# pucedoteth/dora

Measured on AMD Instinct MI355X. Metric: node->node GB/s (40,960,000 B UInt8 samples) + p50/p99 latency per msg size, higher is better.
Workload: dtype u8; 1 GPU; C2: examples/benchmark node->sink edge, device-resident UInt8 samples, 1 node + 1 sink per GPU; msg_bytes=40960000, parallelism=dp1 (one dataflow per GPU)

## Files before the change

### dora_amd/_lib.py

```python
from __future__ import annotations

import ctypes
import os
from ctypes import (POINTER, c_char_p, c_double, c_float, c_int, c_int32, c_int64, c_size_t,
                    c_uint8, c_uint32, c_uint64, c_void_p)

from .arrow_c import ArrowArray, ArrowSchema

LIB_DIR = os.path.join(os.path.dirname(os.path.abspath(__file__)), "lib")
LIB_PATH = os.path.join(LIB_DIR, "libdora_gpu.so")
TESTING_PATH = os.path.join(LIB_DIR, "libdora_gpu_testing.so")

ARROW_DEVICE_CPU = 1
ARROW_DEVICE_ROCM = 10
ARROW_DEVICE_ROCM_HOST = 11

DORA_OK = 0
ERRORS = {-1: "invalid", -2: "hip", -3: "too_small", -4: "unsupported", -5: "closed",
          -6: "timeout", -7: "not_found"}


class DoraGpuError(RuntimeError):
    def __init__(self, code, msg):
        super().__init__(f"[{ERRORS.get(code, code)}] {msg}")
# ... 254 lines not shown
                                        POINTER(c_int), POINTER(c_int), POINTER(c_float),
                                        POINTER(c_uint64), POINTER(c_uint64), POINTER(c_uint64)]),
    "dora_gpu_test_plan_quant": (c_int, [c_void_p, c_size_t, POINTER(c_int), POINTER(c_int),
                                         POINTER(c_int), POINTER(c_int)]),
    "dora_gpu_test_plan_take": (c_int, [c_void_p, POINTER(c_int), POINTER(c_void_p),
                                        POINTER(c_uint64), POINTER(c_uint64), POINTER(c_int),
                                        POINTER(ctypes.c_int64), POINTER(ctypes.c_int64),
                                        POINTER(ctypes.c_int64)]),
    "dora_gpu_test_plan_mask": (c_int, [c_void_p, POINTER(c_int), POINTER(c_void_p),
                                        POINTER(c_uint64), POINTER(ctypes.c_int64),
                                        POINTER(ctypes.c_int64), POINTER(c_uint64),
                                        POINTER(c_uint64), POINTER(ctypes.c_int64)]),
    "dora_gpu_test_plan_launch": (c_int, [c_void_p, POINTER(c_int), POINTER(c_int),
                                          POINTER(c_int)]),
    "dora_gpu_test_aql_hold": (c_int, [c_int, c_int]),
    "dora_gpu_test_reduce_timeout": (c_int, [c_uint64]),
    "dora_gpu_test_d2h_copy_probe": (c_int, [c_int, c_int, c_uint64, c_uint32, c_uint64, c_void_p]),
    "dora_gpu_test_stream_order_probe": (c_int, [c_int, c_int, c_uint64, c_uint32, c_void_p]),
    "dora_gpu_test_abandoned_slots": (c_int, [c_int, POINTER(c_uint32)]),
    "dora_gpu_test_publish_kernel": (c_int, [c_void_p, c_size_t, c_uint64, POINTER(FillTicket),
                                             c_uint32, c_uint32, c_void_p]),
    "dora_gpu_test_keep_awake_stats": (c_int, [c_int, POINTER(c_uint64), POINTER(c_int)]),
    "dora_gpu_test_aql_ring_wc": (c_int, [c_int, ctypes.POINTER(c_int), ctypes.POINTER(c_int)]),
    "dora_gpu_test_bcast_group": (c_int, [c_int, c_void_p, c_uint64, POINTER(c_int),
                                          POINTER(c_int)]),
    "dora_gpu_test_l1_stale": (c_int, [c_int, c_int, POINTER(c_uint32), POINTER(c_uint32),
                                       POINTER(c_uint32)]),
    "dora_gpu_test_ide_output": (c_int, [c_char_p, c_char_p, c_char_p, c_void_p, c_size_t,
                                         c_void_p, c_size_t, c_uint64, c_uint64, c_void_p,
                                         c_void_p, c_size_t, c_int, c_void_p, c_size_t,
# ... 69 lines not shown
```

### dora_amd/csrc/aql.cpp

```cpp
#include "aql.h"

#include <hip/hip_runtime_api.h>
#include <hsa/hsa.h>
#include <hsa/amd_hsa_signal.h>
#include <hsa/hsa_ext_amd.h>
#include <immintrin.h>
#include <pthread.h>
#include <sys/prctl.h>

#include <algorithm>
#include <chrono>
#include <condition_variable>
#include <cstdio>
#include <cstdlib>
#include <cstring>
#include <deque>
#include <mutex>
#include <string>
#include <thread>
#include <vector>

#include "common.h"
#include "shm.h"

// ... 214 lines not shown
}

void on_queue_error(hsa_status_t st, hsa_queue_t*, void* data) {
  const char* m = nullptr;
  hsa_status_string(st, &m);
  std::fprintf(stderr, "dora-gpu: AQL pack queue error: %s\n", m ? m : "?");
  static_cast<AqlQueue*>(data)->failed.store(true);
}

AqlQueue* create(int device) {
  auto note = [&](const char* what) {
    if (std::getenv("DORA_GPU_TRACE"))
      std::fprintf(stderr, "dora-gpu: AQL dispatch off on device %d: %s\n", device, what);
    return nullptr;
  };
  int bus = 0, dev = 0, dom = 0;
  if (hipDeviceGetAttribute(&bus, hipDeviceAttributePciBusId, device) != hipSuccess ||
      hipDeviceGetAttribute(&dev, hipDeviceAttributePciDeviceId, device) != hipSuccess ||
      hipDeviceGetAttribute(&dom, hipDeviceAttributePciDomainID, device) != hipSuccess)
    return note("PCI location");
  if (hsa_init() != HSA_STATUS_SUCCESS) return note("hsa_init");
  Agents f;
  f.bdf = (uint32_t(bus) << 8) | (uint32_t(dev) << 3);
  f.domain = uint32_t(dom);
  hsa_iterate_agents(on_agent, &f);
  if (!f.gpu_ok || !f.cpu_ok) return note("agent");
  if (f.matches != 1) return note("several GPU agents at the device's PCI location");
  hsa_amd_agent_iterate_memory_pools(f.gpu, on_pool, &f);
  if (!f.pool_ok) return note("device memory pool");
  auto* a = new AqlQueue();
  a->gpu = f.gpu;
  a->device = device;
  hsa_amd_hdp_flush_t hdp{};
  if (hsa_agent_get_info(f.gpu, static_cast<hsa_agent_info_t>(HSA_AMD_AGENT_INFO_HDP_FLUSH),
                         &hdp) != HSA_STATUS_SUCCESS ||
      !hdp.HDP_MEM_FLUSH_CNTL) {
    delete a;
    return note("HDP flush register");
  }
  a->hdp = hdp.HDP_MEM_FLUSH_CNTL;
  hsa_code_object_reader_t reader;
  hsa_executable_t exe;
  const size_t co_size = size_t(dora_aql_code_object_end - dora_aql_code_object);
  if (hsa_code_object_reader_create_from_memory(dora_aql_code_object, co_size, &reader) !=
          HSA_STATUS_SUCCESS ||
      hsa_executable_create_alt(HSA_PROFILE_FULL, HSA_DEFAULT_FLOAT_ROUNDING_MODE_DEFAULT,
                                nullptr, &exe) != HSA_STATUS_SUCCESS ||
      hsa_executable_load_agent_code_object(exe, f.gpu, reader, nullptr, nullptr) !=
          HSA_STATUS_SUCCESS ||
      hsa_executable_freeze(exe, nullptr) != HSA_STATUS_SUCCESS) {
    delete a;
    return note("code object");
  }
  for (int k = 0; k < kKernels; ++k) {
    hsa_executable_symbol_t sym;
    uint32_t ka = 0;
    const std::string sym_name = std::string(kKernelNames[k]) + ".kd";
    if (hsa_executable_get_symbol_by_name(exe, sym_name.c_str(), &f.gpu, &sym) != HSA_STATUS_SUCCESS ||
        hsa_executable_symbol_get_info(sym, HSA_EXECUTABLE_SYMBOL_INFO_KERNEL_OBJECT,
                                       &a->kobj[k]) != HSA_STATUS_SUCCESS ||
        hsa_executable_symbol_get_info(sym, HSA_EXECUTABLE_SYMBOL_INFO_KERNEL_KERNARG_SEGMENT_SIZE,
                                       &ka) != HSA_STATUS_SUCCESS ||
        hsa_executable_symbol_get_info(sym, HSA_EXECUTABLE_SYMBOL_INFO_KERNEL_GROUP_SEGMENT_SIZE,
                                       &a->group[k]) != HSA_STATUS_SUCCESS ||
        hsa_executable_symbol_get_info(
            sym, HSA_EXECUTABLE_SYMBOL_INFO_KERNEL_PRIVATE_SEGMENT_SIZE, &a->priv[k]) !=
            HSA_STATUS_SUCCESS ||
        ka != (k == kMultiKernel    ? aql_args_size()
               : k == kBatchKernel  ? aql_batch_args_size()
               : k == kReduceKernel ? size_t(kReduceArgsBytes)
               : k == kReadKernel   ? size_t(kReadArgsBytes)
                                    : size_t(kArgs1Bytes)) ||
        ka > kSlotBytes) {
      delete a;
      return note("kernel symbol / argument size");
    }
  }
  void* ring = nullptr;
  if (hsa_amd_memory_pool_allocate(f.pool, size_t(kRingSlots) * kSlotBytes, 0, &ring) !=
          HSA_STATUS_SUCCESS ||
      hsa_amd_agents_allow_access(1, &f.cpu, nullptr, ring) != HSA_STATUS_SUCCESS) {
    delete a;
    return note("argument ring");
  }
  a->ring = static_cast<uint8_t*>(ring);
  std::vector<uint8_t> zero(kSlotBytes, 0);
  for (uint32_t r = 0; r < kRingSlots; ++r)
    std::memcpy(a->ring + size_t(r) * kSlotBytes, zero.data(), kSlotBytes);
  __builtin_ia32_sfence();
  (void)*reinterpret_cast<volatile uint32_t*>(a->ring + size_t(kRingSlots - 1) * kSlotBytes);
  const int create_queues = std::min(kMaxQueues, kQueues);
  for (int i = 0; i < create_queues; ++i) {
    if (hsa_queue_create(f.gpu, kQueuePackets, HSA_QUEUE_TYPE_SINGLE, on_queue_error, a,
                         UINT32_MAX, UINT32_MAX, &a->qs[i]) != HSA_STATUS_SUCCESS)
      break;
    a->nq = i + 1;
  }
  if (a->nq > 0) {
    hsa_amd_pointer_info_t pi{};
    pi.size = sizeof(pi);
    if (hsa_amd_pointer_info(a->qs[0]->base_address, &pi, nullptr, nullptr, nullptr) ==
        HSA_STATUS_SUCCESS) {
      const int owner = pi.agentOwner.handle == f.cpu.handle   ? 1
                        : pi.agentOwner.handle == f.gpu.handle ? 2
                        : pi.agentOwner.handle                  ? 3
                                                                : 0;
      a->ring_where = int(pi.type) * 4 + owner;
      a->wc_ring = owner == 2;
    }
  }
  if (a->nq == 0) {
    hsa_amd_memory_pool_free(ring);
    delete a;
    return note("queue");
  }
  hsa_amd_agent_iterate_memory_pools(f.cpu, on_cpu_pool, &f);
  void* hr = nullptr;
  if (f.kernarg_ok &&
      hsa_amd_memory_pool_allocate(f.kernarg, size_t(kRingSlots) * kHostSlotBytes, 0, &hr) ==
          HSA_STATUS_SUCCESS) {
    if (hsa_amd_agents_allow_access(1, &f.gpu, nullptr, hr) == HSA_STATUS_SUCCESS) {
      std::memset(hr, 0, size_t(kRingSlots) * kHostSlotBytes);
      a->hring = static_cast<uint8_t*>(hr);
    } else {
      hsa_amd_memory_pool_free(hr);
    }
  }
  hsa_system_get_info(HSA_SYSTEM_INFO_TIMESTAMP_FREQUENCY, &a->ts_freq);
  a->cpu = f.cpu;
  std::pair<hsa_amd_memory_pool_t, bool> coarse{{}, false};
  hsa_amd_agent_iterate_memory_pools(f.gpu, on_coarse_pool, &coarse);
  a->coarse = coarse.first;
  a->coarse_ok = coarse.second;
  return a;
}

}

namespace {
void warm_main(AqlQueue* a);
void stop_warm_threads();
std::mutex g_queues_mu;
AqlQueue* g_queues[64] = {};
}

AqlQueue* aql_queue(int device) {
  static std::mutex& mu = g_queues_mu;
  static AqlQueue** queues = g_queues;
  static bool tried[64] = {};
  if (device < 0 || device >= 64) return nullptr;
  std::lock_guard<std::mutex> g(mu);
  if (!tried[device]) {
    tried[device] = true;
    queues[device] = create(device);
    if (queues[device]) {
      queues[device]->warm_thread = std::thread(warm_main, queues[device]);
      static std::once_flag once;
      std::call_once(once, [] {
        std::atexit(stop_warm_threads);
        pthread_atfork(nullptr, nullptr, [] {
          for (AqlQueue* q : g_queues)
            if (q && q->warm_thread.joinable()) {
              new (&q->warm_thread) std::thread();
              q->warm_stop.store(true);
            }
        });
      });
    }
  }
  AqlQueue* q = queues[device];
  return (q && !q->failed.load()) ? q : nullptr;
}

bool aql_usable(const AqlQueue* q) { return q && !q->failed.load(std::memory_order_relaxed); }

size_t aql_max_segments() { return 8; }

namespace {
void drain_backlog(AqlQueue* a, std::chrono::steady_clock::time_point t0,
                   std::chrono::steady_clock::duration limit) {
  for (;;) {
    {
      std::lock_guard<std::mutex> g(a->mu);
      if (a->backlog.empty() || a->failed.load()) return;
    }
    if (std::chrono::steady_clock::now() - t0 > limit) return;
    std::this_thread::yield();
  }
// ... 8 lines not shown
  }
  const auto t0 = std::chrono::steady_clock::now();
  for (AqlQueue* a : qs) {
    if (!a) continue;
    drain_backlog(a, t0, std::chrono::seconds(5));
    std::lock_guard<std::mutex> g(a->mu);
    if (a->fallback) (void)hipStreamSynchronize(a->fallback);
    for (Use& u : a->uses)
      while (u.flag && !fill_reached(u.flag, u.epoch) &&
             std::chrono::steady_clock::now() - t0 < std::chrono::seconds(5))
        __builtin_ia32_pause();
  }
}

void aql_forget_flags(int device, const void* base, size_t size) {
  AqlQueue* a = aql_queue(device);
  if (!a) return;
  const auto t0 = std::chrono::steady_clock::now();
  drain_backlog(a, t0, std::chrono::seconds(2));
  std::lock_guard<std::mutex> g(a->mu);
  if (a->fallback) (void)hipStreamSynchronize(a->fallback);
  const auto* lo = static_cast<const uint8_t*>(base);
  std::deque<Pending> keep_backlog;
  for (const Pending& p : a->backlog) {
    const auto* f = reinterpret_cast<const uint8_t*>(p.flag_host);
    if (f < lo || f >= lo + size) keep_backlog.push_back(p);
  }
  a->backlog.swap(keep_backlog);
  for (auto& o : a->outq) {
    std::deque<Use> keep;
    for (const Use& u : o) {
      const auto* f = reinterpret_cast<const uint8_t*>(u.flag);
// ... 823 lines not shown
```

### dora_amd/csrc/aql.h

```cpp
#pragma once

#include <atomic>
#include <cstddef>
#include <cstdint>

#include "plan.h"

namespace dora {

struct AqlQueue;

AqlQueue* aql_queue(int device);
bool aql_usable(const AqlQueue* q);

int aql_pack(AqlQueue* q, const Segment* segs, size_t n, uint8_t* dst, const FillSignal& sig,
             const std::atomic<uint64_t>* flag_host, bool profile, uint64_t dst_cap = 0,
             uint64_t* cp_stamps = nullptr, bool sync = false, bool* read_signalled = nullptr);
bool aql_cp_candidate(const Segment* segs, size_t n, bool lone = false);

void aql_forget_flags(int device, const void* base, size_t size);

void aql_fence_all();

size_t aql_kernel_count();
const char* aql_kernel_name(size_t k);
uint64_t aql_dispatched(int device, size_t k);
int aql_hold(int device, bool hold);
// ... 29 lines not shown
```

### dora_amd/csrc/node.cpp

```cpp
#include "node_internal.h"

namespace dora {
namespace {

constexpr uint64_t kDropWaitNs = 10000000000;

bool numa_pinning() {
  static const bool v = [] {
    const char* e = std::getenv("DORA_GPU_PIN");
    return !(e && *e == '0');
  }();
  return v;
}

int gpu_numa_node(int device) {
  char bus[64] = {0};
  if (hipDeviceGetPCIBusId(bus, sizeof(bus), device) != hipSuccess) return -1;
  for (char* p = bus; *p; ++p) *p = char(std::tolower(*p));
  const std::string path = std::string("/sys/bus/pci/devices/") + bus + "/numa_node";
  FILE* f = std::fopen(path.c_str(), "r");
  if (!f) return -1;
  int numa = -1;
  if (std::fscanf(f, "%d", &numa) != 1) numa = -1;
  std::fclose(f);
// ... 68 lines not shown
    hipStream_t st = nullptr;
    if (hipStreamCreateWithFlags(&st, hipStreamNonBlocking) != hipSuccess) {
      (void)hipGetLastError();
      c->bcast_error = "broadcast stream of output `" + o + "`";
      continue;
    }
    if (bcast_join(uid, static_cast<int>(nranks), 0, 30000, &comm) == DORA_OK) {
      n->bcast_out[o] = {comm, st};
    } else {
      c->bcast_error = dora_gpu_last_error();
      (void)hipStreamDestroy(st);
    }
  }
}

}
}

extern "C" {

int dora_node_init(const char* shm_name, const char* node_id, int device, dora_node** out) {
  if (!shm_name || !node_id || !out) return dora::fail(DORA_ERR_INVALID, "NULL argument");
  *out = nullptr;
  DORA_GUARD_BEGIN
  auto core = std::make_shared<dora::NodeCore>();
  try {
    core->region.reset(dora::Region::attach(shm_name));
  } catch (const std::exception& e) {
    return dora::fail(DORA_ERR_INVALID, "attach dataflow: %s", e.what());
  }
  core->idx = core->region->node_index(node_id);
// ... 43 lines not shown
    }
  }

  auto* n = new dora_node();
  n->pin_pending = device < 0 && dora::numa_pinning();
  if (const char* e = std::getenv("DORA_GPU_SEND_ASYNC")) n->async_default = *e == '1';
  n->core = core;
  n->id = node_id;
  for (auto& o : dora::split(e.outputs, ',')) n->outputs.insert(o);
  for (auto& kv : dora::split(e.inputs, ',')) {
    auto eq = kv.find('=');
    n->queue_size[kv.substr(0, eq)] = static_cast<uint32_t>(std::stoul(kv.substr(eq + 1)));
  }
  n->min_queue_size = SIZE_MAX;
  for (auto& kv : n->queue_size) n->min_queue_size = std::min<size_t>(n->min_queue_size, kv.second);
  int rc = core->request(dora::REQ_SUBSCRIBE, {});
  if (rc != DORA_OK) {
    delete n;
    return rc;
  }
  const uint64_t t0 = dora::mono_ns();
  for (;;) {
    uint32_t kind;
    std::vector<uint8_t> p;
    if (core->ev.try_pop(&kind, &p)) {
      if (kind == dora::EV_READY) {
        if (p.size() >= 4) {
          dora::RBuf r(p);
          for (uint32_t k = r.u32(); k > 0; --k) n->host_bound.insert(r.str());
        }
// ... 32 lines not shown
  const char* shm = std::getenv("DORA_GPU_DATAFLOW");
  const char* id = std::getenv("DORA_NODE_ID");
  const char* dev = std::getenv("DORA_GPU_DEVICE");
  if (!shm || !id)
    return dora::fail(DORA_ERR_INVALID,
                      "env variables DORA_GPU_DATAFLOW and DORA_NODE_ID must be set. Are you sure "
                      "the node was started by the dataflow launcher?");
  return dora_node_init(shm, id, dev ? std::atoi(dev) : 0, out);
}

void dora_node_free(dora_node* n) {
  if (!n) return;
  struct Flush {
    ~Flush() { dora::trace_flush(); }
  } flush_trace_at_end;
  dora::stdout_capture_stop(n->stdout_capture);
  n->stdout_capture = nullptr;
  dora::stop_pump(n);
  std::vector<std::string> outs(n->outputs.begin(), n->outputs.end());
  dora::WBuf w;
  w.u32(static_cast<uint32_t>(outs.size()));
  for (auto& o : outs) w.str(o);
  (void)n->core->request(dora::REQ_CLOSE_OUTPUTS, w.data(), w.size());
  n->queue.clear();
  uint64_t t0 = dora::mono_ns();
  while (!n->sent_out.empty() || !n->forwarded.empty()) {
    dora::handle_finished_drop_tokens(n);
    if (n->sent_out.empty() && n->forwarded.empty()) break;
    if (dora::mono_ns() - t0 > dora::kDropWaitNs) break;
    n->core->drops.wait(10000);
// ... 153 lines not shown
```

### dora_amd/csrc/node_internal.h

```cpp

#pragma once
#include <hip/hip_runtime_api.h>
#include <pthread.h>
#include <unistd.h>
#include <x86intrin.h>

#include <algorithm>
#include <chrono>
#include <atomic>
#include <condition_variable>
#include <cstdio>
#include <cstdlib>
#include <cstring>
#include <deque>
#include <map>
#include <memory>
#include <memory_resource>
#include <mutex>
#include <new>
#include <thread>
#include <set>
#include <sstream>
#include <random>
#include <string>
// ... 80 lines not shown
  uint64_t cap = 0;
  uint64_t id = 0;
  hipIpcMemHandle_t handle;
  int flag = -1;
  uint64_t fill_epoch = 0;
  uint64_t region_epoch = 0;
  int region_cp_area = -1;
  hipEvent_t done = nullptr;
  hipIpcEventHandle_t done_handle;
  hipEvent_t use_ev = nullptr;
  bool use_pending = false;
  bool host = false;
  std::string shm_name;
  bool registered = false;
  bool bar = false, bar_tried = false;
};

inline uint64_t slot_bytes(uint64_t len) {
  constexpr uint64_t kSlotGrain = 2ull << 20;
  return (std::max<uint64_t>(len, 1) + kSlotGrain - 1) / kSlotGrain * kSlotGrain;
}

constexpr size_t kFillStreams = 1;

constexpr uint64_t kTimingPeriod = 8;

enum PeerCopyMode { PEER_KERNEL, PEER_SDMA };

struct OwnSlots {
  std::mutex mu;
// ... 422 lines not shown
  std::vector<uint32_t> cp_used;
  hipEvent_t start = nullptr;
  std::vector<hipEvent_t> stop;
  uint64_t packs = 0, bytes = 0;
  void fold(uint64_t a, uint64_t b) {
    if (!a || b < a) return;
    if (!stamped || a < tmin) tmin = a;
    if (!stamped || b > tmax) tmax = b;
    ++stamped;
    if (ticks.size() < 2 * (1u << 16)) {
      ticks.push_back(a);
      ticks.push_back(b);
    }
  }
  ~TimedRegion();
};

struct PlanCache {
  struct Entry {
    std::vector<uint64_t> key;
    dora_plan* plan = nullptr;
    std::vector<uint8_t> ti;
    uint64_t last_use = 0;
  };
  std::vector<Entry> entries;
  std::unordered_map<uint64_t, size_t> index;
  std::vector<uint64_t> key_buf;
  uint64_t clock = 0, hits = 0;
  static uint64_t hash(const std::vector<uint64_t>& key) {
    return fnv1a_words(key.data(), key.size());
// ... 38 lines not shown
  std::unordered_set<dora_sample*> samples_live;
  std::thread pump;
  std::mutex qmu;
  std::condition_variable qcv;
  std::atomic<bool> pump_on{false}, pump_stop{false};
  bool want_pump = false;
  bool pin_pending = false;
  dora::TimedRegion timed;
  dora::PackTiming prof;
  dora::PlanCache plans;
  uint64_t aql_packs = 0, hip_packs = 0;
  uint64_t bar_fills = 0;
  std::set<std::string, std::less<>> host_bound;
  uint64_t host_packs = 0, host_copies = 0;
  bool aql_ready = false;
  uint64_t slots_created = 0, cache_hits = 0, dropped_inputs = 0;
  std::vector<uint8_t> drop_buf;
  std::vector<uint8_t> ev_buf;
  bool compact = false;
  bool async_default = false;
  struct BcastOut {
    dora::BcastComm* comm = nullptr;
    hipStream_t stream = nullptr;
  };
  std::map<std::string, BcastOut> bcast_out;
  uint64_t bcast_seq = 0;
  dora::StdoutCapture* stdout_capture = nullptr;
  std::unordered_map<dora::DropToken, std::shared_ptr<dora::InputData>, dora::DropTokenHash>
      forwarded;
  uint64_t zero_copy_forwards = 0;
// ... 11 lines not shown
  if (note == NOTE_NONE) return;
  const std::atomic<uint64_t>* f = c->flag_host(s->slot->flag);
  if (note == NOTE_SYNC_AND_FENCE) NodeCore::note(c->aql_pending, f, epoch);
  NodeCore::note(c->flag_pending, f, epoch);
}

void release_slot_memory(Slot* s);
int self_pid();
bool wait_slot_idle(dora_node* n, Slot* s, uint64_t timeout_ns = kFillWaitNs);
void free_slot(dora_node* n, Slot* s);
void drain_slot_reaper();
void add_to_cache(dora_node* n, Slot* s);
void on_token(dora_node* n, const DropToken& t);
int handle_finished_drop_tokens(dora_node* n);
int allocate_slot(dora_node* n, uint64_t len, Slot** out);
int allocate_host_slot(dora_node* n, uint64_t len, Slot** out);
void discard_sample(dora_node* n, dora_sample* s);
dora_sample* vec_sample(const uint8_t* p, size_t len);
int proxy_send(dora_node* n, const char* output_id, const uint8_t* ti, size_t ti_len,
               const uint8_t* params, size_t params_len, dora_sample* sample, uint64_t ts);
PeerCopyMode peer_copy_mode();
bool edge_copy_forced();
int ensure_peer_access(NodeCore* c, int src_device);
int enqueue_peer_copy(NodeCore* c, void* dst, const void* src, int src_device, uint64_t len);
int ensure_local(InputData* in);
void encode_event(dora_node* n, uint32_t kind, const std::vector<uint8_t>& p);
void start_pump(dora_node* n);
void stop_pump(dora_node* n);
void harvest_region_stamp(dora_node* n, Slot* s);
void ensure_cp_stamps(dora_node* n);

}
```

### dora_amd/csrc/node_measure.cpp

```cpp

#include "node_internal.h"

namespace dora {

void harvest_region_stamp(dora_node* n, Slot* s) {
  const FillFlag& ff = n->core->region->hdr()->nodes[n->core->idx].fill[s->flag];
  if (s->region_cp_area >= 0 && ff.epoch.load(std::memory_order_acquire) != s->region_epoch &&
      ff.cp_epoch.load(std::memory_order_acquire) == s->region_epoch) {
    n->timed.cp_used.push_back(uint32_t(s->region_cp_area));
  } else if (ff.epoch.load(std::memory_order_acquire) == s->region_epoch) {
    n->timed.fold(ff.t_start, ff.t_end);
  }
  s->region_epoch = 0;
  s->region_cp_area = -1;
}

void ensure_cp_stamps(dora_node* n) {
  if (n->timed.cp_stamps || n->core->device < 0) return;
  const size_t bytes = size_t(kRegionCpAreas) * kCpAreaWords * 8;
  void* d = nullptr;
  if (bar_alloc(n->core->device, bytes, &d) != DORA_OK) {
    clear_error();
    return;
  }
  const std::vector<uint8_t> zero(bytes, 0);
  if (bar_write(n->core->device, d, zero.data(), bytes) != DORA_OK) {
    bar_free(d);
    clear_error();
    return;
  }
  n->timed.cp_stamps = static_cast<uint64_t*>(d);
  void* idx = nullptr;
  void* out = nullptr;
  if (hipHostMalloc(&idx, kRegionCpAreas * 4, hipHostMallocCoherent) == hipSuccess &&
      hipHostMalloc(&out, kRegionCpAreas * 16, hipHostMallocCoherent) == hipSuccess) {
    n->timed.reduce_idx = static_cast<uint32_t*>(idx);
    n->timed.reduce_out = static_cast<uint64_t*>(out);
  } else {
    (void)hipGetLastError();
    if (idx) (void)hipHostFree(idx);
  }
}

constexpr size_t kTimingPairs = 64;
constexpr size_t kMaxIntervals = 1 << 16;

void PackTiming::harvest(TimingPair& p) {
  if (!p.pending) return;
  float ms = 0;
  if (hipEventSynchronize(p.stop) == hipSuccess &&
      hipEventElapsedTime(&ms, p.start, p.stop) == hipSuccess) {
    pack_ms += ms;
    ++pack_count;
    pack_bytes += p.bytes;
    float a = 0, b = 0;
    if (timing_ref && intervals.size() < 2 * kMaxIntervals &&
// ... 237 lines not shown
```

### dora_amd/csrc/node_recv.cpp

```cpp

#include "node_internal.h"

namespace dora {

PeerCopyMode peer_copy_mode() {
  static const PeerCopyMode v = [] {
    const char* e = std::getenv("DORA_GPU_PEER_COPY");
    return (e && std::string(e) == "sdma") ? PEER_SDMA : PEER_KERNEL;
  }();
  return v;
}

bool edge_copy_forced() {
  static const bool v = [] {
    const char* e = std::getenv("DORA_GPU_EDGE_COPY");
    return e && *e && *e != '0';
  }();
  return v;
}

namespace {

void join_bcast_group(dora_node* n, const std::string& input, const uint8_t* uid, uint32_t nranks,
                      uint32_t rank) {
// ... 112 lines not shown
          auto it = own_slots().ptrs.find(d.ipc.slot_id);
          if (it != own_slots().ptrs.end()) base = it->second;
        } else {
          IpcKey key;
          std::memcpy(key.b, d.ipc.handle, 64);
          key.pid = d.ipc.owner_pid;
          key.slot = d.ipc.slot_id;
          NodeCore* c = n->core.get();
          std::lock_guard<std::mutex> g(c->ipc_mu);
          auto it = c->ipc_cache.find(key);
          if (it != c->ipc_cache.end()) {
            in->mapping = it->second;
          } else {
            hipIpcMemHandle_t h;
            std::memcpy(&h, d.ipc.handle, sizeof(h));
            DeviceScope ds(c->device >= 0 ? c->device : int(d.ipc.device));
            hipError_t e = hipIpcOpenMemHandle(&base, h, hipIpcMemLazyEnablePeerAccess);
            if (e != hipSuccess) {
              ev->type = DORA_EVENT_ERROR;
              ev->error = std::string("hipIpcOpenMemHandle: ") + hipGetErrorString(e) +
                          " (slot " + std::to_string(d.ipc.slot_id) + " of pid " +
                          std::to_string(d.ipc.owner_pid) + " on GPU " +
                          std::to_string(d.ipc.device) + ", " + std::to_string(d.ipc.len) + " B)";
              base = nullptr;
            } else {
              in->mapping = std::make_shared<IpcMapping>();
              in->mapping->base = base;
              c->ipc_cache.emplace(key, in->mapping);
              c->ipc_opens.fetch_add(1, std::memory_order_relaxed);
              n->core->region->hdr()->nodes[c->idx].ipc_opens.fetch_add(1, std::memory_order_relaxed);
              c->trim_ipc_cache();
// ... 29 lines not shown
      const uint32_t rank = r.u32();
      join_bcast_group(n, input, uid, nranks, rank);
      return;
    }
    default:
      return;
  }
  n->queue.push_back(std::move(ev));
}

namespace {

int stage_to_host(InputData* in, int src_device) {
  NodeCore* c = in->core.get();
  if (in->ext_len) {
    DeviceScope ds(src_device);
    uint64_t cap = 0;
    void* h = c->host_pool.get(in->ext_len, &cap);
    if (!h)
      return fail(DORA_ERR_HIP, "pinned staging buffer of %llu bytes",
                  (unsigned long long)in->ext_len);
    hipError_t e = hipSuccess;
    const int hrc = hsa_copy_host(h, in->ptr, in->ext_len, true);
    if (hrc == DORA_ERR_TIMEOUT) return hrc;
    if (hrc != DORA_OK) {
      static std::atomic<bool> noted{false};
      if (std::getenv("DORA_GPU_TRACE") && !noted.exchange(true))
        std::fprintf(stderr, "dora-gpu: staging through HIP's copy: %s\n", dora_gpu_last_error());
      clear_error();
      hipStream_t st = c->stage_stream(src_device);
      e = st ? hipMemcpyAsync(h, in->ptr, in->ext_len, hipMemcpyDeviceToHost, st)
             : hipErrorInvalidResourceHandle;
      if (e == hipSuccess) e = hipStreamSynchronize(st);
    }
    if (e != hipSuccess) {
      (void)hipGetLastError();
      c->host_pool.put(h, cap);
// ... 450 lines not shown
```

### dora_amd/csrc/node_send.cpp

```cpp

#include "node_internal.h"

namespace dora {
namespace {

constexpr uint64_t kSmallInFlightBytes = 8ull << 20;

size_t max_in_flight(uint64_t len) {
  static const std::pair<long, long> env = [] {
    const char* e = std::getenv("DORA_GPU_MAX_IN_FLIGHT");
    if (!e) return std::make_pair(0L, 0L);
    char* end = nullptr;
    const long a = std::strtol(e, &end, 10);
    const long b = (end && *end == ':') ? std::atol(end + 1) : a;
    return std::make_pair(a, b);
  }();
  const long v = len < kSmallInFlightBytes ? env.first : env.second;
  if (v > 0) return static_cast<size_t>(v);
  return len < kSmallInFlightBytes ? 11 : 8;
}

constexpr uint64_t kSlotWaitNs = 5000000;

void put_metadata(WBuf& w, const std::vector<uint8_t>& ti, const uint8_t* params,
// ... 129 lines not shown
    return DORA_OK;
  }
  if (n->core->device < 0 || (host_inline && std::max(len, ext_len) < kZeroCopyThreshold)) {
    auto* s = new dora_sample();
    s->len = len;
    s->vec.assign(len, 0);
    *out = s;
    return DORA_OK;
  }
  SubSpan sp_new(SP_SAMPLE_NEW);
  auto* s = new dora_sample();
  s->len = len;
  sp_new.stop();
  if (len > 0) {
    if (!n->aql_ready) {
      n->aql_ready = true;
      if (aql_queue(n->core->device)) ensure_cp_stamps(n);
    }
    SubSpan sp_tok(SP_ALLOC_TOKENS);
    handle_finished_drop_tokens(n);
    sp_tok.stop();
    SubSpan sp_wait(SP_ALLOC_WAIT);
    wait_for_send_credit(n, len);
    sp_wait.stop();
    s->ext_len = std::max(len, ext_len);
    SubSpan sp_slot(SP_ALLOC_SLOT);
    int rc = allocate_slot(n, s->ext_len + workspace, &s->slot);
    if (rc != DORA_OK) {
      delete s;
      return rc;
    }
  }
// ... 801 lines not shown
```

### dora_amd/csrc/node_slots.cpp

```cpp

#include "node_internal.h"

namespace dora {
namespace {

constexpr size_t kMaxCacheSize = 20;
constexpr size_t kMaxCacheSlots = 64;
uint64_t slot_cache_bytes() {
  static const uint64_t v = [] {
    const char* e = std::getenv("DORA_GPU_SLOT_CACHE_BYTES");
    return e ? std::strtoull(e, nullptr, 10) : uint64_t(4) << 30;
  }();
  return v;
}

}

void release_slot_memory(Slot* s) {
  if (s->host) {
    if (s->registered) (void)hipHostUnregister(s->ptr);
    shmem_unmap(s->ptr, s->cap);
    shmem_unlink(s->shm_name);
  } else {
    if (s->done) (void)hipEventDestroy(s->done);
// ... 178 lines not shown
    }
  }
  return best;
}

int allocate_slot(dora_node* n, uint64_t len, Slot** out) {
  const int best = best_fit(n, len, slot_bytes(len), false);
  if (best >= 0) {
    Slot* s = n->cache[static_cast<size_t>(best)];
    n->cache.erase(n->cache.begin() + best);
    SubSpan sp_flag(SP_SLOT_FLAG);
    const bool idle = wait_slot_idle(n, s);
    sp_flag.stop();
    if (idle) {
      *out = s;
      ++n->cache_hits;
      return DORA_OK;
    }
    std::fprintf(stderr, "dora-gpu: slot %llu: last fill did not complete; not reused\n",
                 (unsigned long long)s->id);
    std::lock_guard<std::mutex> g(own_slots().mu);
    own_slots().ptrs.erase(s->id);
  }
  auto* s = new Slot();
  s->cap = slot_bytes(len);
  s->id = own_slots().next_id.fetch_add(1);
  DeviceScope ds(n->core->device);
  hipError_t e = hipMalloc(&s->ptr, slot_bytes(len));
  if (e == hipSuccess) e = hipIpcGetMemHandle(&s->handle, s->ptr);
  if (e == hipSuccess) {
    if (n->core->region_dev && !n->core->free_flags.empty()) {
      s->flag = static_cast<int>(n->core->free_flags.back());
      n->core->free_flags.pop_back();
    } else {
      e = hipEventCreateWithFlags(&s->done, hipEventInterprocess | hipEventDisableTiming);
      if (e == hipSuccess) e = hipIpcGetEventHandle(&s->done_handle, s->done);
    }
  }
  if (e != hipSuccess) {
    if (s->flag >= 0) n->core->free_flags.push_back(static_cast<uint32_t>(s->flag));
    if (s->done) (void)hipEventDestroy(s->done);
    if (s->ptr) (void)hipFree(s->ptr);
    delete s;
    return fail(DORA_ERR_HIP, "device slot of %llu bytes: %s", (unsigned long long)len,
                hipGetErrorString(e));
  }
  {
    std::lock_guard<std::mutex> g(own_slots().mu);
    own_slots().ptrs[s->id] = s->ptr;
  }
  ++n->slots_created;
  n->core->region->hdr()->nodes[n->core->idx].slots_created.fetch_add(1, std::memory_order_relaxed);
  *out = s;
  return DORA_OK;
}

int allocate_host_slot(dora_node* n, uint64_t len, Slot** out) {
  constexpr uint64_t kPage = 4096;
  const uint64_t need = (std::max<uint64_t>(len, 1) + kPage - 1) / kPage * kPage;
  const int best = best_fit(n, len, need, true);
  if (best >= 0) {
    *out = n->cache[static_cast<size_t>(best)];
    n->cache.erase(n->cache.begin() + best);
    ++n->cache_hits;
    return DORA_OK;
  }
  auto* s = new Slot();
  s->host = true;
  s->cap = need;
// ... 23 lines not shown
```

### dora_amd/csrc/subprof.h

```cpp
#pragma once

#include <x86intrin.h>

#include <cstdint>

namespace dora {

enum SubPhase : int {
  SP_SEND_PLAN = 0,
  SP_ALLOC_TOKENS,
  SP_ALLOC_WAIT,
  SP_ALLOC_SLOT,
  SP_STREAM_QUERY,
  SP_AQL_PACK,
  SP_AQL_ARGS,
  SP_AQL_DISPATCH,
  SP_SEND_TI,
  SP_SEND_TOKENS,
  SP_SEND_LOOKUP,
  SP_SEND_REQUEST,
  SP_SEND_TRACK,
  SP_RECV_DRAIN,
  SP_RECV_ENCODE,
  SP_RECV_DROPOLD,
// ... 9 lines not shown
extern const bool g_subprof_on;
inline bool subprof_enabled() { return g_subprof_on; }
void subprof_add(int phase, uint64_t ticks);

struct SubSpan {
  int phase;
  uint64_t t0;
  explicit SubSpan(int p) : phase(p), t0(subprof_enabled() ? __rdtsc() : 0) {}
  void stop() {
    if (t0) subprof_add(phase, __rdtsc() - t0);
    t0 = 0;
  }
  ~SubSpan() { stop(); }
};

}
```

### dora_amd/csrc/trace.cpp

```cpp
#include "trace.h"

#include <sched.h>
#include <unistd.h>

#include <atomic>
#include <cstdio>
#include <cstdlib>
#include <cstring>
#include <string>
#include <mutex>
#include <vector>

#include "shm.h"
#include "subprof.h"

namespace dora {
namespace {

struct Rec {
  uint64_t t;
  DropToken tok;
  uint8_t p;
  int16_t cpu;
};
// ... 83 lines not shown
  std::atomic<uint64_t> calls[SP_COUNT] = {};
  uint64_t tsc0 = __rdtsc(), ns0 = mono_ns();
  ~SubProf() {
    if (!on) return;
    const double ns_per_tick = double(mono_ns() - ns0) / double(__rdtsc() - tsc0);
    std::fprintf(stderr, "{\"subphases\": {");
    bool first = true;
    for (int k = 0; k < SP_COUNT; ++k) {
      const uint64_t c = calls[k].load();
      if (!c) continue;
      std::fprintf(stderr, "%s\"%s\": [%.1f, %llu]", first ? "" : ", ", kSubNames[k],
                   double(ticks[k].load()) * ns_per_tick / double(c), (unsigned long long)c);
      first = false;
    }
    std::fprintf(stderr, "}, \"pid\": %d}\n", int(getpid()));
  }
};

SubProf& subprof() {
  static SubProf p;
  return p;
}

}

const bool g_subprof_on = [] {
  const char* e = std::getenv("DORA_GPU_TRACE");
  return e && *e && std::strcmp(e, "0") != 0;
}();

void subprof_add(int phase, uint64_t ticks) {
  SubProf& p = subprof();
  p.ticks[phase].fetch_add(ticks, std::memory_order_relaxed);
  p.calls[phase].fetch_add(1, std::memory_order_relaxed);
}

}
```

### include/dora_gpu_testing.h

```cpp
#ifndef DORA_GPU_TESTING_H
#define DORA_GPU_TESTING_H

#include "dora_gpu.h"

#ifdef __cplusplus
extern "C" {
#endif

int dora_gpu_test_l2_touch(const void* data, size_t len, dora_stream_t stream);
int dora_gpu_test_bar_alloc(int device, size_t bytes, void** out);
int dora_gpu_test_aql_hold(int device, int hold);
int dora_gpu_test_reduce_timeout(uint64_t ns);
int dora_gpu_test_d2h_copy_probe(int device, int mode, uint64_t bytes, uint32_t n,
                                 uint64_t gap_ns, uint64_t* out_ns);
int dora_gpu_test_stream_order_probe(int device, int mode, uint64_t bytes, uint32_t n,
                                     uint64_t* out_ns);
int dora_gpu_test_abandoned_slots(int device, uint32_t* slots);
int dora_gpu_test_publish_kernel(void* dst, size_t len, uint64_t seed,
                                 const dora_fill_ticket* ticket, uint32_t threads_per_wg,
                                 uint32_t store_mode, dora_stream_t stream);
int dora_gpu_test_keep_awake_stats(int device, uint64_t* heartbeats, int* parked);
int dora_gpu_test_aql_ring_wc(int device, int* wc, int* where);
int dora_gpu_test_batch_args(size_t n_msgs, const size_t* seg_counts, const uint64_t* segs,
                             const uint64_t* dsts, const uint64_t* dst_caps,
                             const uint64_t* flags, const uint64_t* epochs, uint8_t* out,
                             size_t cap, uint32_t* grid);
// ... 47 lines not shown
```

Before: 3258 GB/s.

## Prepare AQL queues, CP stamps and first slot on a background thread at node init

At node creation a background thread now builds the AQL queues, the CP stamp areas and one device slot, and the first send joins it and adopts the results instead of doing that setup inline. The goal is to move cold-start setup off the critical path of the first message. Cold-start timing spans are also added under the profiler. The change adds thread lifetime handling (atexit and fork hooks) and a prepared slot sized for a minimal length, which may be too small for large messages and would then be replaced.

Result: slower. 3212 GB/s (-1.4%).

```diff
diff --git a/dora_amd/_lib.py b/dora_amd/_lib.py
--- a/dora_amd/_lib.py
+++ b/dora_amd/_lib.py
@@ -292,6 +292,8 @@
     "dora_gpu_test_plan_launch": (c_int, [c_void_p, POINTER(c_int), POINTER(c_int),
                                           POINTER(c_int)]),
     "dora_gpu_test_aql_hold": (c_int, [c_int, c_int]),
+    "dora_gpu_test_aql_queue_sets": (c_int, [c_int, POINTER(c_int)]),
+    "dora_gpu_test_aql_disable": (c_int, [c_int]),
     "dora_gpu_test_reduce_timeout": (c_int, [c_uint64]),
     "dora_gpu_test_d2h_copy_probe": (c_int, [c_int, c_int, c_uint64, c_uint32, c_uint64, c_void_p]),
     "dora_gpu_test_stream_order_probe": (c_int, [c_int, c_int, c_uint64, c_uint32, c_void_p]),
diff --git a/dora_amd/csrc/aql.cpp b/dora_amd/csrc/aql.cpp
--- a/dora_amd/csrc/aql.cpp
+++ b/dora_amd/csrc/aql.cpp
@@ -252,12 +252,15 @@
       std::fprintf(stderr, "dora-gpu: AQL dispatch off on device %d: %s\n", device, what);
     return nullptr;
   };
+  ColdSpan cs("hip_pci_attrs");
   int bus = 0, dev = 0, dom = 0;
   if (hipDeviceGetAttribute(&bus, hipDeviceAttributePciBusId, device) != hipSuccess ||
       hipDeviceGetAttribute(&dev, hipDeviceAttributePciDeviceId, device) != hipSuccess ||
       hipDeviceGetAttribute(&dom, hipDeviceAttributePciDomainID, device) != hipSuccess)
     return note("PCI location");
+  cs.next("hsa_init");
   if (hsa_init() != HSA_STATUS_SUCCESS) return note("hsa_init");
+  cs.next("agents_pools");
   Agents f;
   f.bdf = (uint32_t(bus) << 8) | (uint32_t(dev) << 3);
   f.domain = uint32_t(dom);
@@ -277,6 +280,7 @@
     return note("HDP flush register");
   }
   a->hdp = hdp.HDP_MEM_FLUSH_CNTL;
+  cs.next("code_object");
   hsa_code_object_reader_t reader;
   hsa_executable_t exe;
   const size_t co_size = size_t(dora_aql_code_object_end - dora_aql_code_object);
@@ -290,6 +294,7 @@
     delete a;
     return note("code object");
   }
+  cs.next("symbols");
   for (int k = 0; k < kKernels; ++k) {
     hsa_executable_symbol_t sym;
     uint32_t ka = 0;
@@ -314,6 +319,7 @@
       return note("kernel symbol / argument size");
     }
   }
+  cs.next("arg_ring");
   void* ring = nullptr;
   if (hsa_amd_memory_pool_allocate(f.pool, size_t(kRingSlots) * kSlotBytes, 0, &ring) !=
           HSA_STATUS_SUCCESS ||
@@ -327,6 +333,7 @@
     std::memcpy(a->ring + size_t(r) * kSlotBytes, zero.data(), kSlotBytes);
   __builtin_ia32_sfence();
   (void)*reinterpret_cast<volatile uint32_t*>(a->ring + size_t(kRingSlots - 1) * kSlotBytes);
+  cs.next("queues");
   const int create_queues = std::min(kMaxQueues, kQueues);
   for (int i = 0; i < create_queues; ++i) {
     if (hsa_queue_create(f.gpu, kQueuePackets, HSA_QUEUE_TYPE_SINGLE, on_queue_error, a,
@@ -352,6 +359,7 @@
     delete a;
     return note("queue");
   }
+  cs.next("host_ring");
   hsa_amd_agent_iterate_memory_pools(f.cpu, on_cpu_pool, &f);
   void* hr = nullptr;
   if (f.kernarg_ok &&
@@ -380,17 +388,20 @@
 void stop_warm_threads();
 std::mutex g_queues_mu;
 AqlQueue* g_queues[64] = {};
+bool g_tried[64] = {};
+std::atomic<int> g_queue_sets[64] = {};
 }
 
 AqlQueue* aql_queue(int device) {
   static std::mutex& mu = g_queues_mu;
   static AqlQueue** queues = g_queues;
-  static bool tried[64] = {};
+  bool* const tried = g_tried;
   if (device < 0 || device >= 64) return nullptr;
   std::lock_guard<std::mutex> g(mu);
   if (!tried[device]) {
     tried[device] = true;
     queues[device] = create(device);
+    if (queues[device]) g_queue_sets[device].fetch_add(1, std::memory_order_relaxed);
     if (queues[device]) {
       queues[device]->warm_thread = std::thread(warm_main, queues[device]);
       static std::once_flag once;
@@ -410,6 +421,28 @@
   return (q && !q->failed.load()) ? q : nullptr;
 }
 
+AqlQueue* aql_queue_if_created(int device) {
+  if (device < 0 || device >= 64) return nullptr;
+  std::lock_guard<std::mutex> g(g_queues_mu);
+  return g_queues[device];
+}
+
+int aql_queue_sets(int device) {
+  if (device < 0 || device >= 64) return 0;
+  return g_queue_sets[device].load(std::memory_order_relaxed);
+}
+
+void aql_stop_warm_threads() { stop_warm_threads(); }
+
+int aql_disable(int device) {
+  if (device < 0 || device >= 64) return fail(DORA_ERR_INVALID, "device %d", device);
+  std::lock_guard<std::mutex> g(g_queues_mu);
+  if (g_tried[device] && g_queues[device])
+    return fail(DORA_ERR_INVALID, "device %d already has AQL queues", device);
+  g_tried[device] = true;
+  return DORA_OK;
+}
+
 bool aql_usable(const AqlQueue* q) { return q && !q->failed.load(std::memory_order_relaxed); }
 
 size_t aql_max_segments() { return 8; }
@@ -448,8 +481,8 @@
 }
 
 void aql_forget_flags(int device, const void* base, size_t size) {
-  AqlQueue* a = aql_queue(device);
-  if (!a) return;
+  AqlQueue* a = aql_queue_if_created(device);
+  if (!a || a->failed.load()) return;
   const auto t0 = std::chrono::steady_clock::now();
   drain_backlog(a, t0, std::chrono::seconds(2));
   std::lock_guard<std::mutex> g(a->mu);
diff --git a/dora_amd/csrc/aql.h b/dora_amd/csrc/aql.h
--- a/dora_amd/csrc/aql.h
+++ b/dora_amd/csrc/aql.h
@@ -11,6 +11,10 @@
 struct AqlQueue;
 
 AqlQueue* aql_queue(int device);
+AqlQueue* aql_queue_if_created(int device);
+int aql_queue_sets(int device);
+void aql_stop_warm_threads();
+int aql_disable(int device);
 bool aql_usable(const AqlQueue* q);
 
 int aql_pack(AqlQueue* q, const Segment* segs, size_t n, uint8_t* dst, const FillSignal& sig,
diff --git a/dora_amd/csrc/node.cpp b/dora_amd/csrc/node.cpp
--- a/dora_amd/csrc/node.cpp
+++ b/dora_amd/csrc/node.cpp
@@ -106,7 +106,90 @@
   }
 }
 
-}
+constexpr size_t kMaxLivePrepares = 64;
+std::atomic<Prepare*> g_live_prepares[kMaxLivePrepares] = {};
+
+bool register_prepare(Prepare* p) {
+  static std::once_flag once;
+  std::call_once(once, [] {
+    std::atexit([] {
+      for (auto& e : g_live_prepares)
+        if (Prepare* q = e.load()) (void)q->join();
+      aql_stop_warm_threads();
+    });
+    pthread_atfork(nullptr, nullptr, [] {
+      for (auto& e : g_live_prepares)
+        if (Prepare* q = e.exchange(nullptr)) new (&q->th) std::thread();
+    });
+  });
+  for (auto& e : g_live_prepares) {
+    Prepare* none = nullptr;
+    if (e.compare_exchange_strong(none, p)) return true;
+  }
+  return false;
+}
+
+void unregister_prepare(Prepare* p) {
+  for (auto& e : g_live_prepares) {
+    Prepare* cur = p;
+    if (e.compare_exchange_strong(cur, nullptr)) return;
+  }
+}
+
+}
+
+void Prepare::start(int dev) {
+  if (dev < 0 || th.joinable() || !register_prepare(this)) return;
+  device = dev;
+  try {
+    th = std::thread([this] {
+      if (hipSetDevice(device) != hipSuccess) {
+        (void)hipGetLastError();
+        return;
+      }
+      queues = aql_queue(device) != nullptr;
+      if (!queues) return;
+      stamps = make_cp_stamps(device);
+      hipError_t e = hipSuccess;
+      slot = make_slot_memory(device, 1, &e);
+      (void)hipGetLastError();
+    });
+  } catch (const std::system_error&) {
+    unregister_prepare(this);
+  }
+}
+
+bool Prepare::join() {
+  if (!th.joinable()) return false;
+  th.join();
+  unregister_prepare(this);
+  return true;
+}
+
+Prepare::~Prepare() {
+  (void)join();
+  free_cp_stamps(stamps);
+  if (slot) {
+    (void)hipFree(slot->ptr);
+    delete slot;
+  }
+}
+
+void join_prepare(dora_node* n) {
+  Prepare& p = n->prep;
+  if (!p.join()) return;
+  n->aql_ready = true;
+  adopt_cp_stamps(n, p.stamps);
+  if (Slot* s = p.slot) {
+    p.slot = nullptr;
+    if (adopt_slot(n, s) == hipSuccess) {
+      s->prepared = true;
+      add_to_cache(n, s);
+    }
+    (void)hipGetLastError();
+  }
+}
+
 }
 
 extern "C" {
@@ -180,6 +263,7 @@
   }
   n->min_queue_size = SIZE_MAX;
   for (auto& kv : n->queue_size) n->min_queue_size = std::min<size_t>(n->min_queue_size, kv.second);
+  if (device >= 0 && !n->outputs.empty()) n->prep.start(device);
   int rc = core->request(dora::REQ_SUBSCRIBE, {});
   if (rc != DORA_OK) {
     delete n;
@@ -242,6 +326,7 @@
   struct Flush {
     ~Flush() { dora::trace_flush(); }
   } flush_trace_at_end;
+  dora::join_prepare(n);
   dora::stdout_capture_stop(n->stdout_capture);
   n->stdout_capture = nullptr;
   dora::stop_pump(n);
diff --git a/dora_amd/csrc/node_internal.h b/dora_amd/csrc/node_internal.h
--- a/dora_amd/csrc/node_internal.h
+++ b/dora_amd/csrc/node_internal.h
@@ -118,6 +118,7 @@
   std::string shm_name;
   bool registered = false;
   bool bar = false, bar_tried = false;
+  bool prepared = false;
 };
 
 inline uint64_t slot_bytes(uint64_t len) {
@@ -570,6 +571,24 @@
     }
   }
   ~TimedRegion();
+};
+
+struct CpStampAreas {
+  uint64_t* stamps = nullptr;
+  uint32_t* reduce_idx = nullptr;
+  uint64_t* reduce_out = nullptr;
+};
+void free_cp_stamps(CpStampAreas& a);
+
+struct Prepare {
+  std::thread th;
+  int device = -1;
+  bool queues = false;
+  CpStampAreas stamps;
+  Slot* slot = nullptr;
+  void start(int device);
+  bool join();
+  ~Prepare();
 };
 
 struct PlanCache {
@@ -638,6 +657,7 @@
   std::set<std::string, std::less<>> host_bound;
   uint64_t host_packs = 0, host_copies = 0;
   bool aql_ready = false;
+  dora::Prepare prep;
   uint64_t slots_created = 0, cache_hits = 0, dropped_inputs = 0;
   std::vector<uint8_t> drop_buf;
   std::vector<uint8_t> ev_buf;
@@ -679,6 +699,10 @@
 void on_token(dora_node* n, const DropToken& t);
 int handle_finished_drop_tokens(dora_node* n);
 int allocate_slot(dora_node* n, uint64_t len, Slot** out);
+Slot* make_slot_memory(int device, uint64_t len, hipError_t* err);
+hipError_t adopt_slot(dora_node* n, Slot* s);
+void count_slot_created(dora_node* n);
+void join_prepare(dora_node* n);
 int allocate_host_slot(dora_node* n, uint64_t len, Slot** out);
 void discard_sample(dora_node* n, dora_sample* s);
 dora_sample* vec_sample(const uint8_t* p, size_t len);
@@ -694,5 +718,7 @@
 void stop_pump(dora_node* n);
 void harvest_region_stamp(dora_node* n, Slot* s);
 void ensure_cp_stamps(dora_node* n);
-
-}
+CpStampAreas make_cp_stamps(int device);
+void adopt_cp_stamps(dora_node* n, CpStampAreas& a);
+
+}
diff --git a/dora_amd/csrc/node_measure.cpp b/dora_amd/csrc/node_measure.cpp
--- a/dora_amd/csrc/node_measure.cpp
+++ b/dora_amd/csrc/node_measure.cpp
@@ -15,31 +15,58 @@
   s->region_cp_area = -1;
 }
 
-void ensure_cp_stamps(dora_node* n) {
-  if (n->timed.cp_stamps || n->core->device < 0) return;
+CpStampAreas make_cp_stamps(int device) {
+  CpStampAreas r;
+  if (device < 0) return r;
   const size_t bytes = size_t(kRegionCpAreas) * kCpAreaWords * 8;
   void* d = nullptr;
-  if (bar_alloc(n->core->device, bytes, &d) != DORA_OK) {
+  ColdSpan cs("cp_stamps_alloc");
+  if (bar_alloc(device, bytes, &d) != DORA_OK) {
     clear_error();
-    return;
-  }
+    return r;
+  }
+  cs.next("cp_stamps_zero");
   const std::vector<uint8_t> zero(bytes, 0);
-  if (bar_write(n->core->device, d, zero.data(), bytes) != DORA_OK) {
+  if (bar_write(device, d, zero.data(), bytes) != DORA_OK) {
     bar_free(d);
     clear_error();
-    return;
-  }
-  n->timed.cp_stamps = static_cast<uint64_t*>(d);
+    return r;
+  }
+  r.stamps = static_cast<uint64_t*>(d);
+  cs.next("cp_stamps_pinned");
   void* idx = nullptr;
   void* out = nullptr;
   if (hipHostMalloc(&idx, kRegionCpAreas * 4, hipHostMallocCoherent) == hipSuccess &&
       hipHostMalloc(&out, kRegionCpAreas * 16, hipHostMallocCoherent) == hipSuccess) {
-    n->timed.reduce_idx = static_cast<uint32_t*>(idx);
-    n->timed.reduce_out = static_cast<uint64_t*>(out);
+    r.reduce_idx = static_cast<uint32_t*>(idx);
+    r.reduce_out = static_cast<uint64_t*>(out);
   } else {
     (void)hipGetLastError();
     if (idx) (void)hipHostFree(idx);
   }
+  return r;
+}
+
+void free_cp_stamps(CpStampAreas& a) {
+  if (a.stamps) bar_free(a.stamps);
+  if (a.reduce_idx) (void)hipHostFree(a.reduce_idx);
+  if (a.reduce_out) (void)hipHostFree(a.reduce_out);
+  a = CpStampAreas{};
+}
+
+void adopt_cp_stamps(dora_node* n, CpStampAreas& a) {
+  if (n->timed.cp_stamps) return free_cp_stamps(a);
+  n->timed.cp_stamps = a.stamps;
+  n->timed.reduce_idx = a.reduce_idx;
+  n->timed.reduce_out = a.reduce_out;
+  a = CpStampAreas{};
+}
+
+void ensure_cp_stamps(dora_node* n) {
+  if (n->timed.cp_stamps || n->core->device < 0) return;
+  DeviceScope ds(n->core->device);
+  CpStampAreas a = make_cp_stamps(n->core->device);
+  adopt_cp_stamps(n, a);
 }
 
 constexpr size_t kTimingPairs = 64;
diff --git a/dora_amd/csrc/node_recv.cpp b/dora_amd/csrc/node_recv.cpp
--- a/dora_amd/csrc/node_recv.cpp
+++ b/dora_amd/csrc/node_recv.cpp
@@ -150,7 +150,9 @@
           } else {
             hipIpcMemHandle_t h;
             std::memcpy(&h, d.ipc.handle, sizeof(h));
+            ColdSpan cs("recv_device_scope");
             DeviceScope ds(c->device >= 0 ? c->device : int(d.ipc.device));
+            cs.next("recv_ipc_open");
             hipError_t e = hipIpcOpenMemHandle(&base, h, hipIpcMemLazyEnablePeerAccess);
             if (e != hipSuccess) {
               ev->type = DORA_EVENT_ERROR;
@@ -210,13 +212,16 @@
 int stage_to_host(InputData* in, int src_device) {
   NodeCore* c = in->core.get();
   if (in->ext_len) {
+    ColdSpan cs("stage_device_scope");
     DeviceScope ds(src_device);
     uint64_t cap = 0;
+    cs.next("stage_pinned_buffer");
     void* h = c->host_pool.get(in->ext_len, &cap);
     if (!h)
       return fail(DORA_ERR_HIP, "pinned staging buffer of %llu bytes",
                   (unsigned long long)in->ext_len);
     hipError_t e = hipSuccess;
+    cs.next("stage_copy");
     const int hrc = hsa_copy_host(h, in->ptr, in->ext_len, true);
     if (hrc == DORA_ERR_TIMEOUT) return hrc;
     if (hrc != DORA_OK) {
diff --git a/dora_amd/csrc/node_send.cpp b/dora_amd/csrc/node_send.cpp
--- a/dora_amd/csrc/node_send.cpp
+++ b/dora_amd/csrc/node_send.cpp
@@ -167,8 +167,13 @@
   sp_new.stop();
   if (len > 0) {
     if (!n->aql_ready) {
-      n->aql_ready = true;
-      if (aql_queue(n->core->device)) ensure_cp_stamps(n);
+      ColdSpan cs("first_sample_join");
+      join_prepare(n);
+      if (!n->aql_ready) {
+        cs.next("first_sample_setup");
+        n->aql_ready = true;
+        if (aql_queue(n->core->device)) ensure_cp_stamps(n);
+      }
     }
     SubSpan sp_tok(SP_ALLOC_TOKENS);
     handle_finished_drop_tokens(n);
diff --git a/dora_amd/csrc/node_slots.cpp b/dora_amd/csrc/node_slots.cpp
--- a/dora_amd/csrc/node_slots.cpp
+++ b/dora_amd/csrc/node_slots.cpp
@@ -216,7 +216,12 @@
     sp_flag.stop();
     if (idle) {
       *out = s;
-      ++n->cache_hits;
+      if (s->prepared) {
+        s->prepared = false;
+        count_slot_created(n);
+      } else {
+        ++n->cache_hits;
+      }
       return DORA_OK;
     }
     std::fprintf(stderr, "dora-gpu: slot %llu: last fill did not complete; not reused\n",
@@ -224,37 +229,59 @@
     std::lock_guard<std::mutex> g(own_slots().mu);
     own_slots().ptrs.erase(s->id);
   }
+  hipError_t e = hipSuccess;
+  Slot* s = make_slot_memory(n->core->device, len, &e);
+  if (s) e = adopt_slot(n, s);
+  if (e != hipSuccess)
+    return fail(DORA_ERR_HIP, "device slot of %llu bytes: %s", (unsigned long long)len,
+                hipGetErrorString(e));
+  count_slot_created(n);
+  *out = s;
+  return DORA_OK;
+}
+
+Slot* make_slot_memory(int device, uint64_t len, hipError_t* err) {
   auto* s = new Slot();
   s->cap = slot_bytes(len);
   s->id = own_slots().next_id.fetch_add(1);
-  DeviceScope ds(n->core->device);
+  DeviceScope ds(device);
+  ColdSpan cs("slot_malloc");
   hipError_t e = hipMalloc(&s->ptr, slot_bytes(len));
+  cs.next("slot_ipc_export");
   if (e == hipSuccess) e = hipIpcGetMemHandle(&s->handle, s->ptr);
-  if (e == hipSuccess) {
-    if (n->core->region_dev && !n->core->free_flags.empty()) {
-      s->flag = static_cast<int>(n->core->free_flags.back());
-      n->core->free_flags.pop_back();
-    } else {
-      e = hipEventCreateWithFlags(&s->done, hipEventInterprocess | hipEventDisableTiming);
-      if (e == hipSuccess) e = hipIpcGetEventHandle(&s->done_handle, s->done);
-    }
-  }
   if (e != hipSuccess) {
-    if (s->flag >= 0) n->core->free_flags.push_back(static_cast<uint32_t>(s->flag));
-    if (s->done) (void)hipEventDestroy(s->done);
     if (s->ptr) (void)hipFree(s->ptr);
     delete s;
-    return fail(DORA_ERR_HIP, "device slot of %llu bytes: %s", (unsigned long long)len,
-                hipGetErrorString(e));
-  }
-  {
-    std::lock_guard<std::mutex> g(own_slots().mu);
-    own_slots().ptrs[s->id] = s->ptr;
-  }
+    *err = e;
+    return nullptr;
+  }
+  return s;
+}
+
+hipError_t adopt_slot(dora_node* n, Slot* s) {
+  hipError_t e = hipSuccess;
+  if (n->core->region_dev && !n->core->free_flags.empty()) {
+    s->flag = static_cast<int>(n->core->free_flags.back());
+    n->core->free_flags.pop_back();
+  } else {
+    DeviceScope ds(n->core->device);
+    e = hipEventCreateWithFlags(&s->done, hipEventInterprocess | hipEventDisableTiming);
+    if (e == hipSuccess) e = hipIpcGetEventHandle(&s->done_handle, s->done);
+  }
+  if (e != hipSuccess) {
+    if (s->done) (void)hipEventDestroy(s->done);
+    (void)hipFree(s->ptr);
+    delete s;
+    return e;
+  }
+  std::lock_guard<std::mutex> g(own_slots().mu);
+  own_slots().ptrs[s->id] = s->ptr;
+  return hipSuccess;
+}
+
+void count_slot_created(dora_node* n) {
   ++n->slots_created;
   n->core->region->hdr()->nodes[n->core->idx].slots_created.fetch_add(1, std::memory_order_relaxed);
-  *out = s;
-  return DORA_OK;
 }
 
 int allocate_host_slot(dora_node* n, uint64_t len, Slot** out) {
diff --git a/dora_amd/csrc/subprof.h b/dora_amd/csrc/subprof.h
--- a/dora_amd/csrc/subprof.h
+++ b/dora_amd/csrc/subprof.h
@@ -47,4 +47,22 @@
   ~SubSpan() { stop(); }
 };
 
+void cold_note(const char* step, uint64_t ticks);
+
+struct ColdSpan {
+  const char* step;
+  uint64_t t0;
+  explicit ColdSpan(const char* s) : step(s), t0(subprof_enabled() ? __rdtsc() : 0) {}
+  void next(const char* s) {
+    if (!t0) return;
+    const uint64_t t = __rdtsc();
+    cold_note(step, t - t0);
+    step = s;
+    t0 = t;
+  }
+  ~ColdSpan() {
+    if (t0) cold_note(step, __rdtsc() - t0);
+  }
+};
+
 }
diff --git a/dora_amd/csrc/trace.cpp b/dora_amd/csrc/trace.cpp
--- a/dora_amd/csrc/trace.cpp
+++ b/dora_amd/csrc/trace.cpp
@@ -121,7 +121,16 @@
       first = false;
     }
     std::fprintf(stderr, "}, \"pid\": %d}\n", int(getpid()));
+    std::lock_guard<std::mutex> g(cold_mu);
+    if (cold.empty()) return;
+    std::fprintf(stderr, "{\"cold_start\": {");
+    for (size_t k = 0; k < cold.size(); ++k)
+      std::fprintf(stderr, "%s\"%s\": %.0f", k ? ", " : "", cold[k].first,
+                   double(cold[k].second) * ns_per_tick);
+    std::fprintf(stderr, "}, \"pid\": %d}\n", int(getpid()));
   }
+  std::mutex cold_mu;
+  std::vector<std::pair<const char*, uint64_t>> cold;
 };
 
 SubProf& subprof() {
@@ -142,4 +151,15 @@
   p.calls[phase].fetch_add(1, std::memory_order_relaxed);
 }
 
+void cold_note(const char* step, uint64_t ticks) {
+  SubProf& p = subprof();
+  std::lock_guard<std::mutex> g(p.cold_mu);
+  for (auto& kv : p.cold)
+    if (std::strcmp(kv.first, step) == 0) {
+      kv.second += ticks;
+      return;
+    }
+  p.cold.emplace_back(step, ticks);
 }
+
+}
diff --git a/include/dora_gpu_testing.h b/include/dora_gpu_testing.h
--- a/include/dora_gpu_testing.h
+++ b/include/dora_gpu_testing.h
@@ -10,6 +10,8 @@
 int dora_gpu_test_l2_touch(const void* data, size_t len, dora_stream_t stream);
 int dora_gpu_test_bar_alloc(int device, size_t bytes, void** out);
 int dora_gpu_test_aql_hold(int device, int hold);
+int dora_gpu_test_aql_queue_sets(int device, int* sets);
+int dora_gpu_test_aql_disable(int device);
 int dora_gpu_test_reduce_timeout(uint64_t ns);
 int dora_gpu_test_d2h_copy_probe(int device, int mode, uint64_t bytes, uint32_t n,
                                  uint64_t gap_ns, uint64_t* out_ns);
```
